# nschejtman/deepLoopCloser

Hardware: AMD Instinct MI355X
Metric: query-frames/sec vs N-keyframe DB + top-k recall@1 (higher is better)
Workload: dtype bf16; 1 GPU; 1000000 x 4096 bf16 keyframe DB, Q=256, top-20 cosine match, 1 GPU(s); db_rows=1000000, dim=4096, k=20, rows_per_gpu=1000000, pipelined=False, crowded=False

## Files before the change

deeploopcloser_amd/_lib.py:

```python
import ctypes as C
import os

_HERE = os.path.dirname(os.path.abspath(__file__))
LIB_PATH = os.path.join(_HERE, "libdlc_hip.so")

DLC_OK = 0
DLC_ERR_BAD_ARG, DLC_ERR_BAD_SHAPE, DLC_ERR_UNSUPPORTED, DLC_ERR_HIP, DLC_ERR_WORKSPACE = -1, -2, -3, -4, -5
DLC_BF16, DLC_F16, DLC_F32, DLC_F64, DLC_I8, DLC_U8, DLC_I64 = 0, 1, 2, 3, 4, 5, 6
DLC_ACT_NONE, DLC_ACT_SIGMOID, DLC_ACT_RELU = 0, 1, 2
DLC_B_KN, DLC_B_NK = 0, 1
DLC_MAX_K = 128
DLC_MAX_STEP = 8
DLC_ABI_VERSION = 20
DLC_SELECT_COOP, DLC_SELECT_NO_HINTS = 1, 2
DLC_SIM_FORCE_F64, DLC_SIM_NO_HOST_SYNC = 1, 2

_vp, _i64, _int, _sz, _dbl, _flt = C.c_void_p, C.c_int64, C.c_int, C.c_size_t, C.c_double, C.c_float

SIGNATURES = {
    "dlc_abi_version": (_int, []),
    "dlc_create": (_int, [_int, C.POINTER(_vp)]),
    "dlc_destroy": (_int, [_vp]),
    "dlc_last_error": (C.c_char_p, [_vp]),
    "dlc_status_string": (C.c_char_p, [_int]),
    "dlc_gemm_bias_act": (_int, [_vp, _int, _int, _int, _i64, _i64, _i64, _vp, _i64, _vp, _i64, _vp, _vp, _i64, _vp]),
    "dlc_bias_act": (_int, [_vp, _int, _int, _i64, _i64, _vp, _i64, _vp, _vp, _i64, _vp]),
    "dlc_sdav_encode_workspace_bytes": (_sz, [_i64, C.POINTER(_i64), _int, _int]),
    "dlc_sdav_encode": (_int, [_vp, _int, _i64, _int, C.POINTER(_i64), _vp, C.POINTER(_vp), C.POINTER(_vp), _vp, _vp,
                               _sz, _vp]),
# ... 86 lines not shown
    "dlc_cosine_rescore_topk": (_int, [_vp, _int, _vp, _i64, _i64, _vp, _i64, _i64, _i64, _int, _i64, _vp, _vp, _vp, _int,
                                      _vp, _vp, _vp, _vp, _int, _vp]),
    "dlc_cosine_exhaustive_topk": (_int, [_vp, _int, _vp, _i64, _i64, _vp, _i64, _i64, _i64, _int, _i64, _vp, _i64, _dbl,
                                         _vp, _vp, _vp, _vp, _vp, _vp, _sz, _vp]),
    "dlc_topk_merge_strided": (_int, [_vp, _vp, _i64, _vp, _i64, _int, _i64, _int, _vp, _dbl, _vp, _vp, _vp, _vp, _vp, _vp]),
    "dlc_topk_merge": (_int, [_vp, _vp, _vp, _int, _i64, _int, _vp, _vp, _vp, _vp]),
    "dlc_topk_keep_older": (_int, [_vp, _vp, _vp, _i64, _int, _i64, _int, _vp, _vp, _vp]),
    "dlc_cosine_scores_workspace_bytes": (_sz, [_i64, _i64, _i64]),
    "dlc_cosine_scores": (_int, [_vp, _int, _vp, _i64, _i64, _vp, _i64, _i64, _i64, _vp, _i64, _vp, _sz, _vp]),
    "dlc_cosine_score_rows": (_int, [_vp, _int, _vp, _i64, _i64, _vp, _i64, _i64, _i64, _i64, _i64, _vp, _vp, _i64, _vp]),
    "dlc_host_to_device": (_int, [_vp, _vp, _vp, _sz, _vp]),
    "dlc_device_to_host": (_int, [_vp, _vp, _vp, _sz, _vp]),
    "dlc_set_host_threads": (_int, [_vp, _int]),
    "dlc_set_scratch": (_int, [_vp, _vp, _sz]),
    "dlc_set_profiling": (_int, [_vp, _int]),
    "dlc_profile_gemm_ms": (_int, [_vp, C.POINTER(_flt), _int]),
}

_lib = None


class DlcError(RuntimeError):
    """A HIP-side failure (DLC_ERR_HIP / DLC_ERR_WORKSPACE) reported by the C ABI."""


def load():
    global _lib
    if _lib is not None:
        return _lib
    if not os.path.exists(LIB_PATH):
# ... 24 lines not shown
```

deeploopcloser_amd/csrc/api.hip:

```cpp
#include "dlc_internal.h"

#include <new>

extern "C" int dlc_abi_version(void) { return DLC_ABI_VERSION; }

extern "C" const char* dlc_status_string(int status) {
    switch (status) {
        case DLC_OK: return "ok";
        case DLC_ERR_BAD_ARG: return "bad argument";
        case DLC_ERR_BAD_SHAPE: return "bad shape";
        case DLC_ERR_UNSUPPORTED: return "unsupported dtype or mode";
        case DLC_ERR_HIP: return "HIP runtime error";
        case DLC_ERR_WORKSPACE: return "workspace too small";
        default: return "unknown status";
    }
}

extern "C" int dlc_create(int device, dlc_ctx** out) {
    if (!out) return DLC_ERR_BAD_ARG;
    *out = nullptr;
    int count = 0;
    if (hipGetDeviceCount(&count) != hipSuccess || count < 1) return DLC_ERR_HIP;
    if (device < 0 || device >= count) return DLC_ERR_BAD_ARG;
    dlc_ctx* c = new (std::nothrow) dlc_ctx;
// ... 54 lines not shown
    if (!ctx) return DLC_ERR_BAD_ARG;
    if ((scratch && bytes == 0) || ((uintptr_t)scratch & 255))
        return dlc::fail(ctx, DLC_ERR_BAD_ARG, "set_scratch: need a 256-byte aligned buffer (or NULL, 0)");
    ctx->scratch = scratch;
    ctx->scratch_bytes = scratch ? bytes : 0;
    return DLC_OK;
}

extern "C" int dlc_set_profiling(dlc_ctx* ctx, int enabled) {
    if (!ctx) return DLC_ERR_BAD_ARG;
    ctx->profiling = enabled ? 1 : 0;
    ctx->prof_calls = 0;
    return DLC_OK;
}

extern "C" int dlc_profile_gemm_ms(dlc_ctx* ctx, float* out_ms, int capacity) {
    if (!ctx) return DLC_ERR_BAD_ARG;
    if (!out_ms || capacity < 1) return dlc::fail(ctx, DLC_ERR_BAD_ARG, "profile_gemm_ms: bad output");
    dlc::DeviceGuard guard(ctx->device);
    long long n = ctx->prof_calls;
    if (n > DLC_PROFILE_RING) n = DLC_PROFILE_RING;
    if (n > capacity) n = capacity;
    for (long long i = 0; i < n; ++i) {
        const long long call = ctx->prof_calls - n + i;
        const int slot = (int)(call % DLC_PROFILE_RING);
        DLC_HIP_CHECK(ctx, hipEventSynchronize(ctx->ev_stop[slot]));
        float ms = 0.f;
        DLC_HIP_CHECK(ctx, hipEventElapsedTime(&ms, ctx->ev_start[slot], ctx->ev_stop[slot]));
        out_ms[i] = ms;
    }
// ... 3 lines not shown
```

deeploopcloser_amd/csrc/cosine_topk.hip:

```cpp
#include "dlc_internal.h"
#include "lds_dma.h"

#include <algorithm>

namespace {

constexpr int BM = 256;
constexpr int BNQ = 256;
constexpr int BK = 64;
constexpr int NTHREADS = 512;
constexpr int TILE_BYTES = 256 * BK * 2;
constexpr int A_TILE = TILE_BYTES;
constexpr int B_TILE = TILE_BYTES;
#ifndef DLC_A_STAGES
#define DLC_A_STAGES 2
#endif
constexpr int A_STAGES = DLC_A_STAGES;
constexpr int B_RING = A_STAGES * A_TILE;
constexpr int LDS_BYTES = A_STAGES * A_TILE + 2 * B_TILE;
#ifndef DLC_STAGGER_SLEEP
#define DLC_STAGGER_SLEEP 15
#endif
#ifndef DLC_STAGGER_PHASES
#define DLC_STAGGER_PHASES 32
// ... 10 lines not shown
        return __builtin_amdgcn_mfma_f32_16x16x32_bf16(__builtin_bit_cast(bf16x8_t, a),
                                                       __builtin_bit_cast(bf16x8_t, b), c, 0, 0, 0);
    }
    static __device__ __forceinline__ float to_f32(unsigned short h) { return dlc_bf16_bits_to_f32(h); }
};
template <> struct Mfma16<dlc_f16_tag> {
    static __device__ __forceinline__ f32x4_t run(u32x4_t a, u32x4_t b, f32x4_t c) {
        return __builtin_amdgcn_mfma_f32_16x16x32_f16(__builtin_bit_cast(f16x8_t, a),
                                                      __builtin_bit_cast(f16x8_t, b), c, 0, 0, 0);
    }
    static __device__ __forceinline__ float to_f32(unsigned short h) { return dlc_f16_bits_to_f32(h); }
};

__device__ __forceinline__ int swz_a(int r) { return ((r >> 1) & 1) | (((r >> 4) & 3) << 1); }
__device__ __forceinline__ int swz_b(int r) { return (r >> 1) & 7; }

struct alignas(8) HintEntry {
    float r2;
    int id;
};

struct GemmArgs {
    const char* Q;
    const char* DB;
    long long ldq_b;
    long long lddb_b;
    int q;
    long long n;
    int nk;
    float* gmax;
// ... 1 lines not shown
    float* tmax;
    long long ldt;
    HintEntry* hint;
    long long ng;
    long long nh;
    float* S;
    long long lds;
    int stagger_mult;
    int stagger_phases;
    int nqb;
    long long ntiles;
    int nsplit;
    int kchunk;
    float* P;
    long long ldp;
};

constexpr int GEMM_GROUPS = 0;
constexpr int GEMM_DENSE = 1;
constexpr int GEMM_PARTIAL = 2;

constexpr int HALF_BYTES = 128 * 128;

#ifndef DLC_A_CACHE_POLICY
#define DLC_A_CACHE_POLICY " nt"
#endif
DLC_DMA_S_FORM(dma_s_stream, DLC_A_CACHE_POLICY)

template <typename Tag, int MODE, bool MASKQ>
__global__ __launch_bounds__(NTHREADS, 2) void score_gemm_kernel(GemmArgs p) {
// ... 167 lines not shown
        }
    } else if constexpr (MODE == GEMM_DENSE) {
#pragma unroll
        for (int c = 0; c < 4; ++c) {
            const int qidx = qblk * BNQ + wc * 64 + c * 16 + i;
            if (qidx >= p.q) continue;
#pragma unroll
            for (int t = 0; t < 8; ++t) {
                const long long row0 = tile * BM + wr * 128 + (t >> 2) * 64 + 16 * lg + 4 * (t & 3);
#pragma unroll
                for (int r = 0; r < 4; ++r)
                    if (row0 + r < p.n) p.S[(long long)qidx * p.lds + row0 + r] = acc[t][c][r];
            }
        }
    } else {
#pragma unroll
        for (int c = 0; c < 4; ++c) {
            const int qidx = qblk * BNQ + wc * 64 + c * 16 + i;
            float hm[2], gm[2][2];
#pragma unroll
            for (int th = 0; th < 2; ++th) {
                float m0 = acc[th * 4][c][0], m1 = acc[th * 4 + 2][c][0];
#pragma unroll
                for (int tt = 0; tt < 2; ++tt)
#pragma unroll
                    for (int r = 0; r < 4; ++r) {
                        m0 = fmaxf(m0, acc[th * 4 + tt][c][r]);
                        m1 = fmaxf(m1, acc[th * 4 + 2 + tt][c][r]);
                    }
                hm[th] = fmaxf(m0, m1);
                gm[th][0] = m0; gm[th][1] = m1;
                const long long g = tile * (BM / GROUP) + wr * 16 + th * 8 + lg * 2;
                if (qidx < p.q) {
                    float* dst = p.gmax + (long long)qidx * p.ldg + g;
                    if (g + 1 < p.ng) *(float2*)dst = make_float2(m0, m1);
                    else if (g < p.ng) dst[0] = m0;
                }
            }
            float h = fmaxf(hm[0], hm[1]);
            h = fmaxf(h, __shfl_xor(h, 16));
            h = fmaxf(h, __shfl_xor(h, 32));
            const long long ht = tile * 2 + wr;
            if (lg == 0 && qidx < p.q && ht < p.nh) p.tmax[(long long)qidx * p.ldt + ht] = h;
            int rank = 16;
            if (gm[1][1] == h) rank = 9 + lg * 2;
            if (gm[1][0] == h) rank = 8 + lg * 2;
            if (gm[0][1] == h) rank = 1 + lg * 2;
            if (gm[0][0] == h) rank = lg * 2;
            rank = min(rank, __shfl_xor(rank, 16));
            rank = min(rank, __shfl_xor(rank, 32));
            const bool hi_th = (rank & 8) != 0, hi_j = (rank & 1) != 0;
            float v[GROUP];
#pragma unroll
            for (int tt = 0; tt < 2; ++tt)
#pragma unroll
                for (int r = 0; r < 4; ++r) {
                    const float lo = hi_j ? acc[2 + tt][c][r] : acc[tt][c][r];
                    const float hi = hi_j ? acc[6 + tt][c][r] : acc[4 + tt][c][r];
                    v[tt * 4 + r] = hi_th ? hi : lo;
                }
            float first = v[0], second = -INFINITY;
            int astar = GROUP - 1;
#pragma unroll
            for (int r = 1; r < GROUP; ++r) {
                second = __builtin_amdgcn_fmed3f(first, second, v[r]);
                first = fmaxf(first, v[r]);
            }
#pragma unroll
            for (int r = GROUP - 2; r >= 0; --r) astar = v[r] == h ? r : astar;
            const bool none = rank == 16;
            const bool owner = none ? lg == 0 : ((rank >> 1) & 3) == lg;
            if (owner && qidx < p.q && ht < p.nh) {
                HintEntry e;
                e.r2 = none ? INFINITY : second;
                e.id = none ? 0 : ((rank << 3) | astar);
                p.hint[(long long)ht * p.q + qidx] = e;
            }
        }
    }
}

template <typename Tag> struct Dot2;
template <> struct Dot2<dlc_bf16_tag> {
    typedef __attribute__((ext_vector_type(2))) __bf16 v2_t;
    static __device__ __forceinline__ float run(unsigned a, unsigned b, float c) {
        return __builtin_amdgcn_fdot2_f32_bf16(__builtin_bit_cast(v2_t, a), __builtin_bit_cast(v2_t, b), c, false);
    }
};
template <> struct Dot2<dlc_f16_tag> {
    typedef __attribute__((ext_vector_type(2))) _Float16 v2_t;
    static __device__ __forceinline__ float run(unsigned a, unsigned b, float c) {
// ... 64 lines not shown
                m = fmaxf(m, v);
            }
            hmax[qq] = fmaxf(hmax[qq], m);
            if (lane == 0 && qq < p.q && g < p.ng) p.gmax[(long long)qq * p.ldg + g] = m;
        }
    }
    if (lane == 0) {
#pragma unroll
        for (int qq = 0; qq < QB; ++qq) wmax[w][qq] = hmax[qq];
    }
    __syncthreads();
    if (tid < QB && tid < p.q && half < p.nh)
        p.tmax[(long long)tid * p.ldt + half] = fmaxf(fmaxf(wmax[0][tid], wmax[1][tid]), fmaxf(wmax[2][tid], wmax[3][tid]));
}

__device__ __forceinline__ unsigned f32_key(float x) {
    unsigned u = __float_as_uint(x);
    return (u & 0x80000000u) ? ~u : (u | 0x80000000u);
}
__device__ __forceinline__ float key_f32(unsigned k) {
    return __uint_as_float((k & 0x80000000u) ? (k ^ 0x80000000u) : ~k);
}
__device__ __forceinline__ unsigned long long pack_key(float score, unsigned id) {
    return ((unsigned long long)f32_key(score) << 32) | (unsigned long long)(~id);
}
__device__ __forceinline__ unsigned key_id(unsigned long long key) { return ~(unsigned)key; }


__device__ __forceinline__ unsigned wave_max_u32(unsigned v) {
#define DLC_DPP_MAX(ctrl, rmask) \
    v = max(v, (unsigned)__builtin_amdgcn_update_dpp((int)v, (int)v, ctrl, rmask, 0xf, false))
    DLC_DPP_MAX(0x111, 0xf);
    DLC_DPP_MAX(0x112, 0xf);
    DLC_DPP_MAX(0x114, 0xf);
    DLC_DPP_MAX(0x118, 0xf);
    DLC_DPP_MAX(0x142, 0xa);
    DLC_DPP_MAX(0x143, 0xc);
#undef DLC_DPP_MAX
    return (unsigned)__builtin_amdgcn_readlane((int)v, 63);
}

constexpr int FIN_THREADS = 512;
__host__ __device__ inline size_t fin_lds_fixed(int kg) {
    return (size_t)kg * (GROUPS_PER_HALF * 8 + GROUP * (8 + 8 + 4)) + (size_t)(kg + 1) * 8 + 64;
}

__device__ __forceinline__ void rank_select(const unsigned long long* keys, int m, int k, int* out, bool plus_one = false) {
    const int lim = plus_one ? k + 1 : k;
    for (int e = threadIdx.x; e < m; e += blockDim.x) {
        const unsigned long long ke = keys[e];
        if (ke == 0ull) continue;
        int rank = 0;
#pragma unroll 8
        for (int j = 0; j < m; ++j) rank += keys[j] > ke ? 1 : 0;
        if (rank < lim) out[rank] = e;
    }
}
// ... 530 lines not shown
template <typename Tag, int RS_UNROLL, int MODE>
__global__ __launch_bounds__(256) __attribute__((amdgpu_waves_per_eu(5))) void finish_topk_coop_kernel(FinishArgs a) {
    finish_topk_body<Tag, 256, RS_UNROLL, MODE>(a);
}

struct ExhaustiveArgs {
    const float* gmax; long long ldg; long long ng;
    const char* Q; long long ldq_b; const char* DB; long long lddb_b;
    long long n; int d; int k; long long row_offset;
    const double* lower; long long lower_stride;
    float* out_s; double* out_s64; long long* out_i;
    int* status;
    double tau;
    const float* tau_scale;
    int limited; long long limit0;
};
constexpr int EXH_BATCH = 64;
constexpr int EXH_POOL = EXH_BATCH * GROUP + DLC_MAX_K;

template <typename Tag, int RS_UNROLL = 4>
__device__ __forceinline__ void exhaustive_topk_body(const ExhaustiveArgs& a, double lower) {
    const int qi = blockIdx.x;
    __shared__ long long pk[EXH_POOL];
    __shared__ double ps[EXH_POOL];
    __shared__ int pid[EXH_POOL];
    __shared__ int qlist[FIN_THREADS];
    __shared__ int wcnt[FIN_THREADS / 64];
    __shared__ int sel[DLC_MAX_K];
    const int tid = threadIdx.x, lane = tid & 63, w = tid >> 6, k = a.k;
    const long long n_vis = visible_rows(a.n, a.limited, a.limit0, qi);
    const long long ng_vis = a.limited ? (n_vis + GROUP - 1) / GROUP : a.ng;
    const double tau = scaled_tau(a.tau, a.tau_scale, qi);
    double theta = lower - tau;
    int cnt = 0;
    const char* qrow = a.Q + (long long)qi * a.ldq_b;
    for (long long c0 = 0; c0 < ng_vis; c0 += FIN_THREADS) {
        const long long g = c0 + tid;
        const bool qual = g < ng_vis && (double)a.gmax[(long long)qi * a.ldg + g] >= theta;
        const unsigned long long bal = __ballot(qual);
        if (lane == 0) wcnt[w] = __popcll(bal);
        __syncthreads();
        int base = 0, nqual = 0;
#pragma unroll
        for (int ww = 0; ww < FIN_THREADS / 64; ++ww) {
            base += ww < w ? wcnt[ww] : 0;
            nqual += wcnt[ww];
        }
        if (qual) qlist[base + __popcll(bal & ((1ull << lane) - 1ull))] = (int)g;
        __syncthreads();
        for (int b0 = 0; b0 < nqual; b0 += EXH_BATCH) {
            const int nb = min(EXH_BATCH, nqual - b0);
            for (int s = w; s < nb; s += FIN_THREADS / 64) {
                const long long row0 = (long long)qlist[b0 + s] * GROUP;
// ... 30 lines not shown
        }
        __syncthreads();
    }
    for (int e = tid; e < k; e += FIN_THREADS) {
        const bool ok = e < cnt;
        if (a.out_s) a.out_s[(long long)qi * k + e] = ok ? (float)ps[e] : -INFINITY;
        if (a.out_s64) a.out_s64[(long long)qi * k + e] = ok ? ps[e] : -INFINITY;
        a.out_i[(long long)qi * k + e] = ok ? (long long)pid[e] + a.row_offset : -1;
    }
    if (tid == 0) a.status[qi] = 2;
}

template <typename Tag>
__global__ __launch_bounds__(FIN_THREADS) void exhaustive_topk_kernel(ExhaustiveArgs a) {
    const int qi = blockIdx.x;
    if (a.status[qi] != 1) return;
    exhaustive_topk_body<Tag>(a, a.lower[(long long)qi * a.lower_stride]);
}

struct SmallArgs {
    const float* P; long long ldp; long long qstride; int nsplit;
    float* gmax; long long ldg;
    const char* Q; long long ldq_b; const char* DB; long long lddb_b;
    long long n; int d; int k; int m3max; long long row_offset;
    float* out_s; double* out_s64; long long* out_i; int* status; double tau;
    const float* tau_scale;
    int limited; long long limit0;
};
constexpr int SMALL_KT_MAX = 40;
constexpr int SMALL_GPT = 4;
// ... 149 lines not shown
        const int c = sel[e];
        if (c >= 0) {
            if (a.out_s) a.out_s[(long long)qi * k + e] = (float)cs64[c];
            a.out_s64[(long long)qi * k + e] = cs64[c];
            a.out_i[(long long)qi * k + e] = (long long)crow[c] + a.row_offset;
        }
    }
    const int ck = sel[k - 1];
    const double kth = ck >= 0 ? cs64[ck] : -INFINITY;
    const bool cert = bkey == 0u || (ck >= 0 && kth > (double)key_f32(bkey) + scaled_tau(a.tau, a.tau_scale, qi));
    if (cert) {
        if (tid == 0) a.status[qi] = 0;
        return;
    }
    __syncthreads();
    ExhaustiveArgs e;
    e.gmax = a.gmax; e.ldg = a.ldg; e.ng = ng_all;
    e.Q = a.Q; e.ldq_b = a.ldq_b; e.DB = a.DB; e.lddb_b = a.lddb_b;
    e.n = a.n; e.d = a.d; e.k = k; e.row_offset = a.row_offset;
    e.lower = nullptr; e.lower_stride = 0;
    e.out_s = a.out_s; e.out_s64 = a.out_s64; e.out_i = a.out_i;
    e.status = a.status; e.tau = a.tau; e.tau_scale = a.tau_scale;
    e.limited = a.limited; e.limit0 = a.limit0;
    exhaustive_topk_body<Tag, LONG ? 1 : 4>(e, kth);
}

template <typename Tag>
__global__ __launch_bounds__(FIN_THREADS) void small_topk_kernel(SmallArgs a) {
    small_topk_body<Tag, false>(a);
}
template <typename Tag>
// ... 264 lines not shown
        const int64_t kc = dlc::cdiv(nk, ns), ns_eff = dlc::cdiv(nk, kc);
        if (ns_eff != ns) continue;
        if ((double)ns_eff * part_bytes > (double)(1ll << 30)) break;
        const double t = (double)dlc::cdiv(work * ns_eff, (int64_t)256) * ((double)kc * t_k + t_fix) +
                         2.0 * (double)ns_eff * part_bytes / bytes_per_us + t_launch;
        if (t < best_t * 0.9) {
            best_t = t;
            best = SplitPlan{(int)ns_eff, (int)kc};
        }
    }
    return best;
}

struct WsLayout {
    size_t gmax, tmax, hint, part, status, s64, rs_ids, rs_max, rs_scores, rs_idx, rs_bound, total;
    long long ldg, ldt, ldp;
    int kg;
    SplitPlan sp;
    int rparts;
    bool dense;
    bool hints;
    double tau;
};

inline bool gemv_shape(int64_t q, int64_t nk) {
    const int qb = q <= 1 ? 1 : (q <= 2 ? 2 : 4);
    return q <= GEMV_MAX_Q && (long long)qb * nk * 128 <= GEMV_MAX_LDS;
}

constexpr int64_t DENSE_MAX_ROWS = 16384;
// ... 33 lines not shown
    w.ldp = ntiles * BM;
    w.part = o;
    if (w.sp.nsplit > 1 || w.dense) o += dlc::align_up((size_t)w.sp.nsplit * q * w.ldp * 4, 256);
    w.status = o; o += dlc::align_up((size_t)q * 4, 256);
    w.s64 = o; o += dlc::align_up((size_t)q * k * 8, 256);
    w.rparts = w.dense ? 1 : rescore_parts(q, d, w.kg, k);
    w.rs_ids = w.rs_max = w.rs_scores = w.rs_idx = w.rs_bound = o;
    if (w.rparts > 1) {
        w.rs_ids = o; o += dlc::align_up((size_t)q * w.kg * 4, 256);
        w.rs_max = o; o += dlc::align_up((size_t)q * (w.kg + 1) * 4, 256);
        w.rs_scores = o; o += dlc::align_up((size_t)w.rparts * q * k * 8, 256);
        w.rs_idx = o; o += dlc::align_up((size_t)w.rparts * q * k * 8, 256);
        w.rs_bound = o; o += dlc::align_up((size_t)q * 4, 256);
    }
    w.total = o;
    return w;
}

int check_operands(dlc_ctx* ctx, int dtype, const void* Q, int64_t q, int64_t ldq, const void* DB, int64_t n,
                   int64_t lddb, int64_t d) {
    if (!ctx) return DLC_ERR_BAD_ARG;
    if (dtype != DLC_BF16 && dtype != DLC_F16)
        return dlc::fail(ctx, DLC_ERR_UNSUPPORTED, "cosine match: dtype %d (need DLC_BF16 or DLC_F16)", dtype);
    if (!Q || !DB || q < 1 || n < 1 || d < 1) return dlc::fail(ctx, DLC_ERR_BAD_ARG, "cosine match: null/empty operand");
    if (d % BK != 0) return dlc::fail(ctx, DLC_ERR_BAD_SHAPE, "cosine match: d=%lld must be a multiple of %d", (long long)d, BK);
    if (ldq < d || lddb < d || (ldq % 8) || (lddb % 8))
        return dlc::fail(ctx, DLC_ERR_BAD_SHAPE, "cosine match: row strides must be >= d and multiples of 8 elements");
    if (((uintptr_t)Q & 15) || ((uintptr_t)DB & 15))
        return dlc::fail(ctx, DLC_ERR_BAD_ARG, "cosine match: operands must be 16-byte aligned");
    if (ldq * 2 * 255 + 128 > 0xffffffffll || lddb * 2 * 255 + 128 > 0xffffffffll)
// ... 82 lines not shown
        dim3 grid((unsigned)a.q, (unsigned)dlc::cdiv(groups, (long long)256));
        hipLaunchKernelGGL(splitk_groups_kernel, grid, dim3(256), 0, st, a.P, a.ldp, a.q, a.nsplit, a.gmax, a.ldg, a.ng,
                           a.tmax, a.ldt, a.nh, keep ? 1 : 0);
        DLC_LAUNCH_CHECK(ctx, "splitk_groups_kernel");
    }
    return DLC_OK;
}

}

extern "C" size_t dlc_cosine_topk_workspace_bytes(int64_t q, int64_t n, int64_t d, int k) {
    if (q < 1 || n < 1 || d < BK || k < 1 || k > DLC_MAX_K) return 0;
    return ws_layout(q, n, d, k).total;
}

namespace {

struct MatchCall {
    GemmArgs a;
    WsLayout w;
};

int prepare_match(dlc_ctx* ctx, const char* what, int dtype, const void* Q, int64_t q, int64_t ldq, const void* DB,
                  int64_t n, int64_t lddb, int64_t d, int k, void* workspace, size_t workspace_bytes, MatchCall* mc) {
    int rc = check_operands(ctx, dtype, Q, q, ldq, DB, n, lddb, d);
    if (rc != DLC_OK) return rc;
    if (k < 1 || k > DLC_MAX_K) return dlc::fail(ctx, DLC_ERR_BAD_ARG, "%s: k=%d outside 1..%d", what, k, DLC_MAX_K);
    mc->w = ws_layout(q, n, d, k);
    if (!workspace || workspace_bytes < mc->w.total)
        return dlc::fail(ctx, DLC_ERR_WORKSPACE, "%s: workspace %zu < %zu bytes", what, workspace_bytes, mc->w.total);
    if (((uintptr_t)workspace & 255)) return dlc::fail(ctx, DLC_ERR_BAD_ARG, "%s: workspace must be 256-byte aligned", what);
    char* ws = (char*)workspace;
    GemmArgs& a = mc->a;
    a.Q = (const char*)Q; a.DB = (const char*)DB;
    a.ldq_b = ldq * 2; a.lddb_b = lddb * 2;
    a.q = (int)q; a.n = n; a.nk = (int)(d / BK);
    a.gmax = (float*)(ws + mc->w.gmax); a.ldg = mc->w.ldg;
    a.tmax = (float*)(ws + mc->w.tmax); a.ldt = mc->w.ldt;
    a.hint = (HintEntry*)(ws + mc->w.hint);
    a.ng = dlc::cdiv(n, GROUP); a.nh = dlc::cdiv(n, HALF);
    a.S = nullptr; a.lds = 0;
    a.nsplit = mc->w.sp.nsplit; a.kchunk = mc->w.sp.kchunk;
    a.P = (float*)(ws + mc->w.part); a.ldp = mc->w.ldp;
    return DLC_OK;
}

inline bool small_direct(const MatchCall& mc, int k) {
    return mc.w.dense && mc.a.n <= (int64_t)FIN_THREADS * SMALL_GPT * GROUP && k + DENSE_ROW_SLACK + 1 <= SMALL_KT_MAX;
}

int run_score(dlc_ctx* ctx, int dtype, MatchCall& mc, hipStream_t st, bool partials_only = false) {
    return dlc::profiled(ctx, st, [&]() -> int {
        return (dtype == DLC_BF16) ? launch_scores<dlc_bf16_tag>(ctx, mc.a, false, st, mc.w.dense, partials_only)
                                   : launch_scores<dlc_f16_tag>(ctx, mc.a, false, st, mc.w.dense, partials_only);
    });
}

FinishArgs finish_args(const MatchCall& mc, int k, int64_t n, int64_t d, int64_t q, int64_t row_offset) {
    const GemmArgs& g = mc.a;
    FinishArgs f{};
    f.tmax = g.tmax; f.ldt = g.ldt; f.nh = (int)g.nh;
    f.gmax = g.gmax; f.ldg = g.ldg; f.ng = g.ng;
    f.kg = mc.w.kg;
    f.Q = g.Q; f.ldq_b = g.ldq_b; f.DB = g.DB; f.lddb_b = g.lddb_b;
    f.n = n; f.d = (int)d; f.k = k; f.row_offset = row_offset;
    f.tau = mc.w.tau;
    f.nq = q;
    return f;
}

template <typename Tag, int THREADS, int RS_UNROLL, int MODE>
int launch_finish(dlc_ctx* ctx, FinishArgs f, int64_t q, bool small_lds, hipStream_t st) {
    size_t dsm = fin_lds_fixed(f.kg);
    f.tv_in_lds = MODE != FIN_RESCORE && !small_lds && (size_t)f.nh * 4 <= 96 * 1024;
    if (f.tv_in_lds) dsm += (size_t)f.nh * 4;
    dsm = dlc::align_up(dsm, 16);
    void (*fk)(FinishArgs);
    if constexpr (THREADS == 256) fk = finish_topk_coop_kernel<Tag, RS_UNROLL, MODE>;
    else fk = finish_topk_kernel<Tag, THREADS, RS_UNROLL, MODE>;
    if (dsm > 48 * 1024)
        DLC_HIP_CHECK(ctx, hipFuncSetAttribute((const void*)fk, hipFuncAttributeMaxDynamicSharedMemorySize, (int)dsm));
    hipLaunchKernelGGL(fk, dim3((unsigned)q, (unsigned)(MODE == FIN_RESCORE && f.gparts > 1 ? f.gparts : 1)), dim3(THREADS),
                       dsm, st, f);
    DLC_LAUNCH_CHECK(ctx, "finish_topk_kernel");
    return DLC_OK;
}

template <int MODE>
int run_select(dlc_ctx* ctx, int dtype, const FinishArgs& f, int64_t q, int flags, hipStream_t st) {
    const bool coop = (flags & DLC_SELECT_COOP) != 0;
    if (dtype == DLC_BF16)
        return coop ? launch_finish<dlc_bf16_tag, 256, 1, MODE>(ctx, f, q, true, st)
                    : launch_finish<dlc_bf16_tag, 512, 4, MODE>(ctx, f, q, false, st);
    return coop ? launch_finish<dlc_f16_tag, 256, 1, MODE>(ctx, f, q, true, st)
                : launch_finish<dlc_f16_tag, 512, 4, MODE>(ctx, f, q, false, st);
}

int run_exhaustive(dlc_ctx* ctx, int dtype, const FinishArgs& f, int64_t q, const double* lower, int64_t lower_stride,
                   float* out_s, double* out_s64, int64_t* out_i, int* status, hipStream_t st) {
    ExhaustiveArgs e{};
    e.gmax = f.gmax; e.ldg = f.ldg; e.ng = f.ng;
    e.Q = f.Q; e.ldq_b = f.ldq_b; e.DB = f.DB; e.lddb_b = f.lddb_b;
    e.n = f.n; e.d = f.d; e.k = f.k; e.row_offset = f.row_offset;
    e.lower = lower; e.lower_stride = lower_stride;
    e.out_s = out_s; e.out_s64 = out_s64; e.out_i = (long long*)out_i;
    e.status = status; e.tau = f.tau; e.tau_scale = f.tau_scale;
    e.limited = f.limited; e.limit0 = f.limit0;
    if (dtype == DLC_BF16)
        hipLaunchKernelGGL(exhaustive_topk_kernel<dlc_bf16_tag>, dim3((unsigned)q), dim3(FIN_THREADS), 0, st, e);
    else
        hipLaunchKernelGGL(exhaustive_topk_kernel<dlc_f16_tag>, dim3((unsigned)q), dim3(FIN_THREADS), 0, st, e);
    DLC_LAUNCH_CHECK(ctx, "exhaustive_topk_kernel");
    return DLC_OK;
}

// ... 45 lines not shown
        if (rc != DLC_OK) return rc;
    } else {
        f.grp_ids = (int*)(ws + mc.w.rs_ids); f.grp_max = (float*)(ws + mc.w.rs_max);
        rc = run_select<FIN_GROUPS>(ctx, dtype, f, q, 0, st);
        if (rc != DLC_OK) return rc;
        double* ps = (double*)(ws + mc.w.rs_scores);
        int64_t* pi = (int64_t*)(ws + mc.w.rs_idx);
        float* pb = (float*)(ws + mc.w.rs_bound);
        f.gparts = mc.w.rparts; f.out_s = nullptr; f.out_s64 = ps; f.out_i = (long long*)pi; f.bound_out = pb;
        rc = run_select<FIN_RESCORE>(ctx, dtype, f, q, DLC_SELECT_COOP, st);
        if (rc != DLC_OK) return rc;
        rc = launch_merge(ctx, ps, q * k, pi, q * k, mc.w.rparts, q, k, pb, mc.w.tau, tau_scale, out_scores, s64, out_idx, status, st);
        if (rc != DLC_OK) return rc;
    }
    if (direct) return DLC_OK;
    return run_exhaustive(ctx, dtype, f, q, s64 + (k - 1), k, out_scores, s64, out_idx, status, st);
}

}

extern "C" double dlc_cosine_score_error_bound(int64_t q, int64_t n, int64_t d, int k) {
    if (q < 1 || n < 1 || d < BK || k < 1 || k > DLC_MAX_K) return 0.0;
    return ws_layout(q, n, d, k).tau;
}

extern "C" int dlc_cosine_topk(dlc_ctx* ctx, int dtype, const void* Q, int64_t q, int64_t ldq, const void* DB,
                               int64_t n, int64_t lddb, int64_t d, int k, int64_t row_offset, float* out_scores,
                               double* out_scores_f64, int64_t* out_idx, int32_t* out_status, const float* tau_scale,
                               void* workspace, size_t workspace_bytes, void* stream) {
    if (!ctx) return DLC_ERR_BAD_ARG;
    if (!out_scores || !out_idx) return dlc::fail(ctx, DLC_ERR_BAD_ARG, "cosine_topk: null output");
    MatchCall mc;
    int rc = prepare_match(ctx, "cosine_topk", dtype, Q, q, ldq, DB, n, lddb, d, k, workspace, workspace_bytes, &mc);
    if (rc != DLC_OK) return rc;
    dlc::DeviceGuard guard(ctx->device);
    if (!guard.ok) return dlc::fail(ctx, DLC_ERR_HIP, "hipSetDevice(%d) failed", ctx->device);
    const bool direct = small_direct(mc, k);
    rc = run_score(ctx, dtype, mc, (hipStream_t)stream, direct);
    if (rc != DLC_OK) return rc;
    return run_finish(ctx, dtype, mc, k, n, d, q, row_offset, out_scores, out_scores_f64, out_idx, out_status, workspace, 0,
                      tau_scale, (hipStream_t)stream, 0, 0, direct);
}

extern "C" int dlc_cosine_topk_older(dlc_ctx* ctx, int dtype, const void* Q, int64_t q, int64_t ldq, const void* DB,
                                     int64_t n, int64_t lddb, int64_t d, int k, int64_t row_offset, int64_t limit0,
                                     float* out_scores, double* out_scores_f64, int64_t* out_idx, int32_t* out_status,
                                     const float* tau_scale, void* workspace, size_t workspace_bytes, void* stream) {
    if (!ctx) return DLC_ERR_BAD_ARG;
    if (!out_scores || !out_idx) return dlc::fail(ctx, DLC_ERR_BAD_ARG, "cosine_topk_older: null output");
    MatchCall mc;
    int rc = prepare_match(ctx, "cosine_topk_older", dtype, Q, q, ldq, DB, n, lddb, d, k, workspace, workspace_bytes, &mc);
    if (rc != DLC_OK) return rc;
// ... 345 lines not shown
```

deeploopcloser_amd/csrc/dlc_internal.h:

```cpp
#pragma once
#include <hip/hip_runtime.h>
#include <stdint.h>
#include <stdarg.h>
#include <stdio.h>
#include <string.h>
#include <mutex>

#include "../../include/dlc.h"

struct dlc_host_staging;

struct dlc_ctx {
    int device;
    char err[512];
    int profiling;
    long long prof_calls;
    hipEvent_t ev_start[DLC_PROFILE_RING];
    hipEvent_t ev_stop[DLC_PROFILE_RING];
    void* scratch;
    size_t scratch_bytes;
    unsigned long long func_attr_set;
    void* zero_page;
    dlc_host_staging* staging;
    std::mutex* host_lock;
    int host_threads;
    unsigned long long* host_flag;
    hipEvent_t ev_flag;
};

enum {
    DLC_ATTR_GEMM_BASE = 0,
    DLC_ATTR_GEMV_BASE = 16,
    DLC_ATTR_DGEMM_BASE = 24,
    DLC_ATTR_DMA64_BASE = 32,
    DLC_ATTR_PAIR_TILE = 48,
    DLC_ATTR_GRAM_I8 = 49,
    DLC_ATTR_PAIR_FILTER = 50,
    DLC_ATTR_SPLIT_F16 = 51,
    DLC_ATTR_DS_DMA = 52,
    DLC_ATTR_CONV_SPLIT_F16 = 53,
};

// ... 110 lines not shown
```

deeploopcloser_amd/engine.py:

```python
import collections
import contextlib
import ctypes as C
import weakref

import numpy as np
import torch

from . import _lib as L

_TORCH_TO_DLC = {torch.bfloat16: L.DLC_BF16, torch.float16: L.DLC_F16, torch.float32: L.DLC_F32,
                 torch.float64: L.DLC_F64, torch.int8: L.DLC_I8}
_NAME_TO_TORCH = {"bf16": torch.bfloat16, "bfloat16": torch.bfloat16, "f16": torch.float16, "fp16": torch.float16,
                  "float16": torch.float16, "f32": torch.float32, "float32": torch.float32, "f64": torch.float64,
                  "float64": torch.float64}

SCRATCH_BYTES = 256 << 20
K_STEP = 64


TopK = collections.namedtuple("TopK", "scores idx scores_f64 status")


_RAW_STREAM = getattr(torch._C, "_cuda_getCurrentRawStream", None)

# ... 1086 lines not shown
            raise ValueError("stored descriptors must be 2-D with one width")
        if q.dtype != db.dtype or q.dtype not in (torch.bfloat16, torch.float16):
            raise ValueError("stored descriptors must both be bf16 or both fp16")
        if q.stride(1) != 1 or db.stride(1) != 1:
            raise ValueError("stored descriptor rows must be contiguous")

    def match_topk(self, q, db, k, row_offset=0, out=None, details=False, older_than=None, tau_scale=None):
        self._check_stored(q, db)
        nq, d = q.shape
        if tau_scale is not None:
            self._check_out("tau_scale", tau_scale, (nq,), torch.float32)
        n = db.shape[0]
        need = self.lib.dlc_cosine_topk_workspace_bytes(nq, n, d, k)
        if need == 0:
            raise ValueError("match_topk: k=%d outside 1..%d (or empty operand)" % (k, L.DLC_MAX_K))
        ws = self.workspace("topk", need)
        if out is None:
            scores = torch.empty((nq, k), dtype=torch.float32, device=self.device)
            idx = torch.empty((nq, k), dtype=torch.int64, device=self.device)
        else:
            scores = self._check_out("out[0] (scores)", out[0], (nq, k), torch.float32)
            idx = self._check_out("out[1] (idx)", out[1], (nq, k), torch.int64)
        s64 = torch.empty((nq, k), dtype=torch.float64, device=self.device) if details else None
        status = torch.empty((nq,), dtype=torch.int32, device=self.device) if details else None
        if older_than is None:
            self._check(self.lib.dlc_cosine_topk(self.ctx, _TORCH_TO_DLC[q.dtype], _ptr(q), nq, q.stride(0), _ptr(db), n,
                                                  db.stride(0), d, k, row_offset, _ptr(scores), _ptr(s64), _ptr(idx),
                                                  _ptr(status), _ptr(tau_scale), _ptr(ws), ws.numel(), self._stream()))
        else:
            self._check(self.lib.dlc_cosine_topk_older(self.ctx, _TORCH_TO_DLC[q.dtype], _ptr(q), nq, q.stride(0), _ptr(db), n,
# ... 185 lines not shown
            raise ValueError("cosine_score_rows: empty descriptors")
        ld_out = (o_s if o_s is not None else o_k).stride(0) if nq > 1 else n
        if both and nq > 1 and o_k.stride(0) != ld_out:
            raise ValueError("cosine_score_rows: out and out_keys must have one row stride (%d, %d)" % (ld_out, o_k.stride(0)))
        self._check(self.lib.dlc_cosine_score_rows(self.ctx, _TORCH_TO_DLC[q.dtype], _ptr(q), nq, q.stride(0), _ptr(db), n,
                                                    db.stride(0), d, n if limit0 is None else int(limit0), int(limit_step),
                                                    _ptr(o_s), _ptr(o_k), ld_out, self._stream()))
        for t in (o_s, o_k):
            if t is not None:
                self._wrote(t)
        return ret

    def set_profiling(self, enabled):
        self._check(self.lib.dlc_set_profiling(self.ctx, 1 if enabled else 0))

    def profile_gemm_ms(self, capacity=256):
        buf = (C.c_float * capacity)()
        n = self.lib.dlc_profile_gemm_ms(self.ctx, buf, capacity)
        if n < 0:
            self._check(n)
        return [float(buf[i]) for i in range(n)]


_default = {}


def default_engine(device=None):
    if device is None:
        if not torch.cuda.is_available():
            L.load()
# ... 8 lines not shown
```

include/dlc.h:

```cpp
#ifndef DLC_H_
#define DLC_H_

#include <stddef.h>
#include <stdint.h>

#ifdef __cplusplus
extern "C" {
#endif

#define DLC_ABI_VERSION 20

typedef struct dlc_ctx dlc_ctx;

typedef enum dlc_status {
    DLC_OK = 0,
    DLC_ERR_BAD_ARG = -1,
    DLC_ERR_BAD_SHAPE = -2,
    DLC_ERR_UNSUPPORTED = -3,
    DLC_ERR_HIP = -4,
    DLC_ERR_WORKSPACE = -5
} dlc_status;

typedef enum dlc_dtype {
    DLC_BF16 = 0,
// ... 186 lines not shown
int dlc_contrast_rows(dlc_ctx* ctx, int dtype, const void* scores, int64_t rows, int64_t n, int64_t ld,
                      int64_t limit0, int64_t limit_step, int radius,
                      double* out, int64_t ld_out, void* stream);

size_t dlc_peak_topk_rows_workspace_bytes(int64_t rows, int64_t n, int k);
int dlc_peak_topk_rows(dlc_ctx* ctx, int dtype , const void* scores,
                       int64_t rows, int64_t n, int64_t ld, int64_t limit0, int64_t limit_step,
                       int lower_is_better, int64_t suppress, int has_absent, int64_t absent, int k,
                       void* out_scores, int64_t* out_idx, const int64_t* poison,
                       void* workspace, size_t workspace_bytes, void* stream);

int dlc_l2_normalize_rows(dlc_ctx* ctx, int src_dtype, const void* src, int64_t n, int64_t d, int64_t lds,
                          int center, int dst_dtype, void* dst, int64_t ldd, void* stream);
#define DLC_MAX_K 128
size_t dlc_cosine_topk_workspace_bytes(int64_t q, int64_t n, int64_t d, int k);
int dlc_cosine_topk(dlc_ctx* ctx, int dtype, const void* Q, int64_t q, int64_t ldq,
                    const void* DB, int64_t n, int64_t lddb, int64_t d, int k, int64_t row_offset,
                    float* out_scores, double* out_scores_f64, int64_t* out_idx, int32_t* out_status,
                    const float* tau_scale, void* workspace, size_t workspace_bytes, void* stream);
int dlc_max_row_norm(dlc_ctx* ctx, int dtype, const void* rows, int64_t n, int64_t ld, int64_t d, float* max_norm,
                     void* stream);
int dlc_cosine_tau_scale(dlc_ctx* ctx, int dtype, const void* Q, int64_t q, int64_t ldq, int64_t d,
                         const float* db_max_norm, float* tau_scale, void* stream);
int dlc_cosine_topk_older(dlc_ctx* ctx, int dtype, const void* Q, int64_t q, int64_t ldq,
                          const void* DB, int64_t n, int64_t lddb, int64_t d, int k, int64_t row_offset, int64_t limit0,
                          float* out_scores, double* out_scores_f64, int64_t* out_idx, int32_t* out_status,
                          const float* tau_scale, void* workspace, size_t workspace_bytes, void* stream);
double dlc_cosine_score_error_bound(int64_t q, int64_t n, int64_t d, int k);
double dlc_cosine_score_error_bound_any_plan(int64_t d);
#define DLC_SELECT_COOP 1
// ... 59 lines not shown
```

Before: 126,900 query-frames/s.

## Prune score-tile epilogue writes with a running per-query top-k threshold

```diff
diff --git a/deeploopcloser_amd/_lib.py b/deeploopcloser_amd/_lib.py
--- a/deeploopcloser_amd/_lib.py
+++ b/deeploopcloser_amd/_lib.py
@@ -13,6 +13,7 @@
 DLC_MAX_STEP = 8
 DLC_ABI_VERSION = 20
 DLC_SELECT_COOP, DLC_SELECT_NO_HINTS = 1, 2
+DLC_PRUNE_ON, DLC_PRUNE_OFF, DLC_PRUNE_KEEP = 0, 1, 2
 DLC_SIM_FORCE_F64, DLC_SIM_NO_HOST_SYNC = 1, 2
 
 _vp, _i64, _int, _sz, _dbl, _flt = C.c_void_p, C.c_int64, C.c_int, C.c_size_t, C.c_double, C.c_float
@@ -129,6 +130,8 @@
     "dlc_set_host_threads": (_int, [_vp, _int]),
     "dlc_set_scratch": (_int, [_vp, _vp, _sz]),
     "dlc_set_profiling": (_int, [_vp, _int]),
+    "dlc_set_prune_mode": (_int, [_vp, _int]),
+    "dlc_cosine_topk_prune_bytes": (_sz, [_i64, _i64, _i64, _int]),
     "dlc_profile_gemm_ms": (_int, [_vp, C.POINTER(_flt), _int]),
 }
 
diff --git a/deeploopcloser_amd/csrc/api.hip b/deeploopcloser_amd/csrc/api.hip
--- a/deeploopcloser_amd/csrc/api.hip
+++ b/deeploopcloser_amd/csrc/api.hip
@@ -92,6 +92,15 @@
     return DLC_OK;
 }
 
+extern "C" int dlc_set_prune_mode(dlc_ctx* ctx, int mode) {
+    if (!ctx) return DLC_ERR_BAD_ARG;
+    if (mode != DLC_PRUNE_ON && mode != DLC_PRUNE_OFF && mode != DLC_PRUNE_KEEP)
+        return dlc::fail(ctx, DLC_ERR_BAD_ARG, "set_prune_mode: mode %d", mode);
+    ctx->prune_mode = mode;
+    ctx->prune_kept = 0;
+    return DLC_OK;
+}
+
 extern "C" int dlc_profile_gemm_ms(dlc_ctx* ctx, float* out_ms, int capacity) {
     if (!ctx) return DLC_ERR_BAD_ARG;
     if (!out_ms || capacity < 1) return dlc::fail(ctx, DLC_ERR_BAD_ARG, "profile_gemm_ms: bad output");
diff --git a/deeploopcloser_amd/csrc/cosine_topk.hip b/deeploopcloser_amd/csrc/cosine_topk.hip
--- a/deeploopcloser_amd/csrc/cosine_topk.hip
+++ b/deeploopcloser_amd/csrc/cosine_topk.hip
@@ -48,6 +48,28 @@
 
 __device__ __forceinline__ int swz_a(int r) { return ((r >> 1) & 1) | (((r >> 4) & 3) << 1); }
 __device__ __forceinline__ int swz_b(int r) { return (r >> 1) & 7; }
+
+__device__ __forceinline__ unsigned f32_key(float x) {
+    unsigned u = __float_as_uint(x);
+    return (u & 0x80000000u) ? ~u : (u | 0x80000000u);
+}
+__device__ __forceinline__ float key_f32(unsigned k) {
+    return __uint_as_float((k & 0x80000000u) ? (k ^ 0x80000000u) : ~k);
+}
+
+constexpr int PRUNE_NB = 64;
+constexpr int PRUNE_REFRESH_TILES = 17;
+constexpr int PRUNE_THR_BITS = 20;
+__device__ __forceinline__ unsigned half_key(float h) { return h == -INFINITY ? 0u : f32_key(h); }
+__device__ __forceinline__ unsigned wave_kth_largest_u32(unsigned v, int kt) {
+    unsigned t = 0u;
+#pragma unroll
+    for (int b = 31; b >= 0; --b) {
+        const unsigned c = t | (1u << b);
+        if (__popcll(__ballot(v >= c)) >= kt) t = c;
+    }
+    return t;
+}
 
 struct alignas(8) HintEntry {
     float r2;
@@ -79,6 +101,9 @@
     int kchunk;
     float* P;
     long long ldp;
+    unsigned* bkt;
+    unsigned* thr;
+    int kt;
 };
 
 constexpr int GEMM_GROUPS = 0;
@@ -276,6 +301,13 @@
             }
         }
     } else {
+        const bool prune = p.bkt != nullptr;
+        unsigned thr_seen[4];
+#pragma unroll
+        for (int c = 0; c < 4; ++c) {
+            const int qidx = qblk * BNQ + wc * 64 + c * 16 + i;
+            thr_seen[c] = (prune && qidx < p.q) ? __hip_atomic_load(p.thr + qidx, __ATOMIC_RELAXED, __HIP_MEMORY_SCOPE_AGENT) : 0u;
+        }
 #pragma unroll
         for (int c = 0; c < 4; ++c) {
             const int qidx = qblk * BNQ + wc * 64 + c * 16 + i;
@@ -292,18 +324,30 @@
                     }
                 hm[th] = fmaxf(m0, m1);
                 gm[th][0] = m0; gm[th][1] = m1;
-                const long long g = tile * (BM / GROUP) + wr * 16 + th * 8 + lg * 2;
-                if (qidx < p.q) {
-                    float* dst = p.gmax + (long long)qidx * p.ldg + g;
-                    if (g + 1 < p.ng) *(float2*)dst = make_float2(m0, m1);
-                    else if (g < p.ng) dst[0] = m0;
-                }
             }
             float h = fmaxf(hm[0], hm[1]);
             h = fmaxf(h, __shfl_xor(h, 16));
             h = fmaxf(h, __shfl_xor(h, 32));
             const long long ht = tile * 2 + wr;
-            if (lg == 0 && qidx < p.q && ht < p.nh) p.tmax[(long long)qidx * p.ldt + ht] = h;
+            const bool live = qidx < p.q && ht < p.nh;
+            const unsigned hk = half_key(h);
+            if (lg == 0 && live) {
+                p.tmax[(long long)qidx * p.ldt + ht] = h;
+                if (prune && hk > thr_seen[c])
+                    __hip_atomic_fetch_max(p.bkt + (long long)(ht % PRUNE_NB) * p.q + qidx, hk, __ATOMIC_RELAXED,
+                                           __HIP_MEMORY_SCOPE_AGENT);
+            }
+            const bool pass = !prune || hk >= thr_seen[c] || h != h;
+            if (pass && qidx < p.q) {
+#pragma unroll
+                for (int th = 0; th < 2; ++th) {
+                    const long long g = tile * (BM / GROUP) + wr * 16 + th * 8 + lg * 2;
+                    float* dst = p.gmax + (long long)qidx * p.ldg + g;
+                    if (g + 1 < p.ng) *(float2*)dst = make_float2(gm[th][0], gm[th][1]);
+                    else if (g < p.ng) dst[0] = gm[th][0];
+                }
+            }
+            if (__ballot(pass && live) == 0ull) continue;
             int rank = 16;
             if (gm[1][1] == h) rank = 9 + lg * 2;
             if (gm[1][0] == h) rank = 8 + lg * 2;
@@ -332,11 +376,30 @@
             for (int r = GROUP - 2; r >= 0; --r) astar = v[r] == h ? r : astar;
             const bool none = rank == 16;
             const bool owner = none ? lg == 0 : ((rank >> 1) & 3) == lg;
-            if (owner && qidx < p.q && ht < p.nh) {
+            if (owner && pass && live) {
                 HintEntry e;
                 e.r2 = none ? INFINITY : second;
                 e.id = none ? 0 : ((rank << 3) | astar);
                 p.hint[(long long)ht * p.q + qidx] = e;
+            }
+        }
+        if (prune && tile % PRUNE_REFRESH_TILES == 0) {
+            const int qidx = qblk * BNQ + wid * 64 + lane;
+            if (wid < BNQ / 64 && qidx < p.q) {
+                unsigned v[PRUNE_NB];
+#pragma unroll
+                for (int cl = 0; cl < PRUNE_NB; ++cl)
+                    v[cl] = __hip_atomic_load(p.bkt + (long long)cl * p.q + qidx, __ATOMIC_RELAXED, __HIP_MEMORY_SCOPE_AGENT);
+                unsigned t = 0u;
+#pragma unroll 1
+                for (int b = 31; b >= 32 - PRUNE_THR_BITS; --b) {
+                    const unsigned cand = t | (1u << b);
+                    int cnt = 0;
+#pragma unroll
+                    for (int cl = 0; cl < PRUNE_NB; ++cl) cnt += v[cl] >= cand ? 1 : 0;
+                    if (cnt >= p.kt) t = cand;
+                }
+                if (t != 0u) __hip_atomic_fetch_max(p.thr + qidx, t, __ATOMIC_RELAXED, __HIP_MEMORY_SCOPE_AGENT);
             }
         }
     }
@@ -431,13 +494,6 @@
         p.tmax[(long long)tid * p.ldt + half] = fmaxf(fmaxf(wmax[0][tid], wmax[1][tid]), fmaxf(wmax[2][tid], wmax[3][tid]));
 }
 
-__device__ __forceinline__ unsigned f32_key(float x) {
-    unsigned u = __float_as_uint(x);
-    return (u & 0x80000000u) ? ~u : (u | 0x80000000u);
-}
-__device__ __forceinline__ float key_f32(unsigned k) {
-    return __uint_as_float((k & 0x80000000u) ? (k ^ 0x80000000u) : ~k);
-}
 __device__ __forceinline__ unsigned long long pack_key(float score, unsigned id) {
     return ((unsigned long long)f32_key(score) << 32) | (unsigned long long)(~id);
 }
@@ -458,6 +514,7 @@
 }
 
 constexpr int FIN_THREADS = 512;
+constexpr size_t FIN_TV_LDS_MAX = 96 * 1024;
 __host__ __device__ inline size_t fin_lds_fixed(int kg) {
     return (size_t)kg * (GROUPS_PER_HALF * 8 + GROUP * (8 + 8 + 4)) + (size_t)(kg + 1) * 8 + 64;
 }
@@ -1018,6 +1075,9 @@
     double tau;
     const float* tau_scale;
     int limited; long long limit0;
+    const float* tmax; long long ldt;
+    const unsigned* bkt; unsigned* thr; int kt; long long nq;
+    int publish;
 };
 constexpr int EXH_BATCH = 64;
 constexpr int EXH_POOL = EXH_BATCH * GROUP + DLC_MAX_K;
@@ -1036,11 +1096,23 @@
     const long long ng_vis = a.limited ? (n_vis + GROUP - 1) / GROUP : a.ng;
     const double tau = scaled_tau(a.tau, a.tau_scale, qi);
     double theta = lower - tau;
+    const unsigned thr_final = a.bkt ? wave_kth_largest_u32(a.bkt[(long long)lane * a.nq + qi], a.kt) : 0u;
     int cnt = 0;
     const char* qrow = a.Q + (long long)qi * a.ldq_b;
     for (long long c0 = 0; c0 < ng_vis; c0 += FIN_THREADS) {
         const long long g = c0 + tid;
-        const bool qual = g < ng_vis && (double)a.gmax[(long long)qi * a.ldg + g] >= theta;
+        bool qual = false;
+        if (g < ng_vis) {
+            if (a.bkt) {
+                const float tm = a.tmax[(long long)qi * a.ldt + g / GROUPS_PER_HALF];
+                if (!((double)tm < theta)) {
+                    const bool written = half_key(tm) >= thr_final || tm != tm;
+                    qual = !written || (double)a.gmax[(long long)qi * a.ldg + g] >= theta;
+                }
+            } else {
+                qual = (double)a.gmax[(long long)qi * a.ldg + g] >= theta;
+            }
+        }
         const unsigned long long bal = __ballot(qual);
         if (lane == 0) wcnt[w] = __popcll(bal);
         __syncthreads();
@@ -1101,6 +1173,10 @@
 template <typename Tag>
 __global__ __launch_bounds__(FIN_THREADS) void exhaustive_topk_kernel(ExhaustiveArgs a) {
     const int qi = blockIdx.x;
+    if (a.publish && threadIdx.x < 64) {
+        const unsigned t = wave_kth_largest_u32(a.bkt[(long long)threadIdx.x * a.nq + qi], a.kt);
+        if (threadIdx.x == 0) a.thr[qi] = t;
+    }
     if (a.status[qi] != 1) return;
     exhaustive_topk_body<Tag>(a, a.lower[(long long)qi * a.lower_stride]);
 }
@@ -1280,7 +1356,7 @@
         return;
     }
     __syncthreads();
-    ExhaustiveArgs e;
+    ExhaustiveArgs e{};
     e.gmax = a.gmax; e.ldg = a.ldg; e.ng = ng_all;
     e.Q = a.Q; e.ldq_b = a.ldq_b; e.DB = a.DB; e.lddb_b = a.lddb_b;
     e.n = a.n; e.d = a.d; e.k = k; e.row_offset = a.row_offset;
@@ -1575,6 +1651,8 @@
 
 struct WsLayout {
     size_t gmax, tmax, hint, part, status, s64, rs_ids, rs_max, rs_scores, rs_idx, rs_bound, total;
+    size_t prune, prune_total;
+    bool prunable;
     long long ldg, ldt, ldp;
     int kg;
     SplitPlan sp;
@@ -1638,6 +1716,10 @@
         w.rs_bound = o; o += dlc::align_up((size_t)q * 4, 256);
     }
     w.total = o;
+    w.prunable = w.hints && w.kg <= PRUNE_NB && w.rparts <= 1 && (size_t)dlc::cdiv(n, (int64_t)HALF) * 4 <= FIN_TV_LDS_MAX;
+    w.prune = o;
+    if (w.prunable) o += dlc::align_up((size_t)q * (PRUNE_NB + 1) * 4, 256);
+    w.prune_total = o;
     return w;
 }
 
@@ -1750,11 +1832,18 @@
     return ws_layout(q, n, d, k).total;
 }
 
+extern "C" size_t dlc_cosine_topk_prune_bytes(int64_t q, int64_t n, int64_t d, int k) {
+    if (q < 1 || n < 1 || d < BK || k < 1 || k > DLC_MAX_K) return 0;
+    const WsLayout w = ws_layout(q, n, d, k);
+    return w.prune_total - w.total;
+}
+
 namespace {
 
 struct MatchCall {
     GemmArgs a;
     WsLayout w;
+    bool publish_thr = false;
 };
 
 int prepare_match(dlc_ctx* ctx, const char* what, int dtype, const void* Q, int64_t q, int64_t ldq, const void* DB,
@@ -1778,6 +1867,7 @@
     a.S = nullptr; a.lds = 0;
     a.nsplit = mc->w.sp.nsplit; a.kchunk = mc->w.sp.kchunk;
     a.P = (float*)(ws + mc->w.part); a.ldp = mc->w.ldp;
+    a.bkt = nullptr; a.thr = nullptr; a.kt = 0;
     return DLC_OK;
 }
 
@@ -1808,7 +1898,7 @@
 template <typename Tag, int THREADS, int RS_UNROLL, int MODE>
 int launch_finish(dlc_ctx* ctx, FinishArgs f, int64_t q, bool small_lds, hipStream_t st) {
     size_t dsm = fin_lds_fixed(f.kg);
-    f.tv_in_lds = MODE != FIN_RESCORE && !small_lds && (size_t)f.nh * 4 <= 96 * 1024;
+    f.tv_in_lds = MODE != FIN_RESCORE && !small_lds && (size_t)f.nh * 4 <= FIN_TV_LDS_MAX;
     if (f.tv_in_lds) dsm += (size_t)f.nh * 4;
     dsm = dlc::align_up(dsm, 16);
     void (*fk)(FinishArgs);
@@ -1833,8 +1923,13 @@
 }
 
 int run_exhaustive(dlc_ctx* ctx, int dtype, const FinishArgs& f, int64_t q, const double* lower, int64_t lower_stride,
-                   float* out_s, double* out_s64, int64_t* out_i, int* status, hipStream_t st) {
+                   float* out_s, double* out_s64, int64_t* out_i, int* status, hipStream_t st,
+                   const MatchCall* pruned = nullptr) {
     ExhaustiveArgs e{};
+    if (pruned && pruned->a.bkt) {
+        e.tmax = f.tmax; e.ldt = f.ldt;
+        e.bkt = pruned->a.bkt; e.thr = pruned->a.thr; e.kt = pruned->a.kt; e.nq = pruned->a.q; e.publish = pruned->publish_thr ? 1 : 0;
+    }
     e.gmax = f.gmax; e.ldg = f.ldg; e.ng = f.ng;
     e.Q = f.Q; e.ldq_b = f.ldq_b; e.DB = f.DB; e.lddb_b = f.lddb_b;
     e.n = f.n; e.d = f.d; e.k = f.k; e.row_offset = f.row_offset;
@@ -1910,9 +2005,29 @@
         if (rc != DLC_OK) return rc;
     }
     if (direct) return DLC_OK;
-    return run_exhaustive(ctx, dtype, f, q, s64 + (k - 1), k, out_scores, s64, out_idx, status, st);
-}
-
+    return run_exhaustive(ctx, dtype, f, q, s64 + (k - 1), k, out_scores, s64, out_idx, status, st, &mc);
+}
+
+}
+
+int arm_prune(dlc_ctx* ctx, MatchCall& mc, void* workspace, size_t workspace_bytes, hipStream_t st) {
+    if (ctx->prune_mode == DLC_PRUNE_OFF || !mc.w.prunable || workspace_bytes < mc.w.prune_total) return DLC_OK;
+    GemmArgs& a = mc.a;
+    a.bkt = (unsigned*)((char*)workspace + mc.w.prune);
+    a.thr = a.bkt + (size_t)a.q * PRUNE_NB;
+    a.kt = (int)std::min<long long>(mc.w.kg, a.nh);
+    bool clear = true;
+    if (ctx->prune_mode == DLC_PRUNE_KEEP) {
+        const void* id[3] = {workspace, a.Q, a.DB};
+        const long long shape[4] = {a.q, a.n, a.nk, mc.w.kg};
+        clear = !ctx->prune_kept || memcmp(id, ctx->prune_id, sizeof(id)) != 0 || memcmp(shape, ctx->prune_shape, sizeof(shape)) != 0;
+        memcpy(ctx->prune_id, id, sizeof(id));
+        memcpy(ctx->prune_shape, shape, sizeof(shape));
+        ctx->prune_kept = 1;
+        mc.publish_thr = true;
+    }
+    if (clear) DLC_HIP_CHECK(ctx, hipMemsetAsync(a.bkt, 0, (size_t)a.q * (PRUNE_NB + 1) * 4, st));
+    return DLC_OK;
 }
 
 extern "C" double dlc_cosine_score_error_bound(int64_t q, int64_t n, int64_t d, int k) {
@@ -1932,6 +2047,8 @@
     dlc::DeviceGuard guard(ctx->device);
     if (!guard.ok) return dlc::fail(ctx, DLC_ERR_HIP, "hipSetDevice(%d) failed", ctx->device);
     const bool direct = small_direct(mc, k);
+    rc = arm_prune(ctx, mc, workspace, workspace_bytes, (hipStream_t)stream);
+    if (rc != DLC_OK) return rc;
     rc = run_score(ctx, dtype, mc, (hipStream_t)stream, direct);
     if (rc != DLC_OK) return rc;
     return run_finish(ctx, dtype, mc, k, n, d, q, row_offset, out_scores, out_scores_f64, out_idx, out_status, workspace, 0,
diff --git a/deeploopcloser_amd/csrc/dlc_internal.h b/deeploopcloser_amd/csrc/dlc_internal.h
--- a/deeploopcloser_amd/csrc/dlc_internal.h
+++ b/deeploopcloser_amd/csrc/dlc_internal.h
@@ -26,6 +26,10 @@
     int host_threads;
     unsigned long long* host_flag;
     hipEvent_t ev_flag;
+    int prune_mode;
+    int prune_kept;
+    const void* prune_id[3];
+    long long prune_shape[4];
 };
 
 enum {
diff --git a/deeploopcloser_amd/engine.py b/deeploopcloser_amd/engine.py
--- a/deeploopcloser_amd/engine.py
+++ b/deeploopcloser_amd/engine.py
@@ -1124,6 +1124,8 @@
         need = self.lib.dlc_cosine_topk_workspace_bytes(nq, n, d, k)
         if need == 0:
             raise ValueError("match_topk: k=%d outside 1..%d (or empty operand)" % (k, L.DLC_MAX_K))
+        if older_than is None:
+            need += self.lib.dlc_cosine_topk_prune_bytes(nq, n, d, k)
         ws = self.workspace("topk", need)
         if out is None:
             scores = torch.empty((nq, k), dtype=torch.float32, device=self.device)
@@ -1339,6 +1341,10 @@
     def set_profiling(self, enabled):
         self._check(self.lib.dlc_set_profiling(self.ctx, 1 if enabled else 0))
 
+    def set_prune_mode(self, mode):
+        self._check(self.lib.dlc_set_prune_mode(self.ctx, {"on": L.DLC_PRUNE_ON, "off": L.DLC_PRUNE_OFF,
+                                                           "keep": L.DLC_PRUNE_KEEP}[mode]))
+
     def profile_gemm_ms(self, capacity=256):
         buf = (C.c_float * capacity)()
         n = self.lib.dlc_profile_gemm_ms(self.ctx, buf, capacity)
diff --git a/include/dlc.h b/include/dlc.h
--- a/include/dlc.h
+++ b/include/dlc.h
@@ -224,6 +224,11 @@
                           int center, int dst_dtype, void* dst, int64_t ldd, void* stream);
 #define DLC_MAX_K 128
 size_t dlc_cosine_topk_workspace_bytes(int64_t q, int64_t n, int64_t d, int k);
+#define DLC_PRUNE_ON 0
+#define DLC_PRUNE_OFF 1
+#define DLC_PRUNE_KEEP 2
+size_t dlc_cosine_topk_prune_bytes(int64_t q, int64_t n, int64_t d, int k);
+int dlc_set_prune_mode(dlc_ctx* ctx, int mode);
 int dlc_cosine_topk(dlc_ctx* ctx, int dtype, const void* Q, int64_t q, int64_t ldq,
                     const void* DB, int64_t n, int64_t lddb, int64_t d, int k, int64_t row_offset,
                     float* out_scores, double* out_scores_f64, int64_t* out_idx, int32_t* out_status,
```

Measured after the change: 129,500 query-frames/s (median of 6 runs). 2.0% higher.
